# CSB5/lofreq

Hardware: AMD Instinct MI355X
Metric: pileup columns/sec at depth 10000 (higher is better)
Workload: dtype f64

## Files before the change

lofreq_amd/csrc/lfq_api.hip:

```cpp
#include "lfq_bound.h"
#include "lfq_ctx.h"

namespace {

struct LfqDeviceStreams {
    hipStream_t stream = nullptr, dps = nullptr, side[2] = {nullptr, nullptr};
    hipEvent_t ev_tail[3] = {nullptr, nullptr, nullptr};
    bool tail_recorded = false;
    hipEvent_t ev_end = nullptr;
    bool end_recorded = false;
    int refs = 0;
};
std::mutex g_streams_m;
LfqDeviceStreams g_streams[64];

bool acquire_streams(int device, lfq_ctx *c);
void release_streams(int device);

void *pin_acquire_impl(lfq_ctx *c, size_t bytes, int *slot)
{
    int best = -1, empty = -1, smallest = -1;
    for (int i = 0; i < LFQ_PIN_SLOTS; i++) {
        auto &b = c->pin_pool[i];
        if (b.used) {
// ... 230 lines not shown
    (void)hipSetDevice(c->device);
    for (;;) {
        {
            std::unique_lock<std::mutex> lk(*c->lm);
            c->lcv->wait(lk, [&] { return c->leader_go > 0 || c->leader_stop; });
            if (c->leader_stop) {
                return;
            }
            c->leader_go--;
        }
        int64_t n = 0;
        if (hipEventSynchronize(c->ev_heavy) == hipSuccess) {
            n = std::min<int64_t>(std::max<int64_t>(*(volatile int32_t *)c->h_nheavy, 0), c->heavy_cap);
        }
        lfq_sb_precompute(c->h_tuples, 3 * n);
        {
            std::lock_guard<std::mutex> lk(*c->lm);
            c->sb_pending--;
        }
        c->lcv->notify_all();
    }
}

int ensure_workspace(lfq_ctx *c, int64_t ncols)
{
    if (ncols > c->ws_cols) {
        int64_t cap = 0;
        int64_t want = ncols + ncols / 8 + 1024;
        if (c->d_flags) (void)hipFree(c->d_flags);
        if (c->d_prefix) (void)hipFree(c->d_prefix);
        if (c->d_entries) (void)hipFree(c->d_entries);
        if (c->d_tiles) (void)hipFree(c->d_tiles);
        if (c->d_unsplit) (void)hipFree(c->d_unsplit);
        if (c->d_retry) (void)hipFree(c->d_retry);
        c->d_unsplit = nullptr;
        c->d_retry = nullptr;
        c->d_flags = nullptr;
        c->d_prefix = nullptr;
        c->d_entries = nullptr;
        c->d_tiles = nullptr;
        c->ws_cols = 0;
        LFQ_TRY(grow(&c->d_flags, &cap, want));
        cap = 0;
        LFQ_TRY(grow(&c->d_prefix, &cap, want));
        cap = 0;
        LFQ_TRY(grow(&c->d_entries, &cap, want));
        cap = 0;
        LFQ_TRY(grow(&c->d_tiles, &cap, 2 * (want / 1024 + 8 * (LFQ_MAX_SEGMENTS + 1))));
        cap = 0;
        LFQ_TRY(grow(&c->d_unsplit, &cap, want));
        cap = 0;
        LFQ_TRY(grow(&c->d_retry, &cap, want));
        c->ws_cols = want;
    }
    return LFQ_OK;
}


}

void *lfq_pin_acquire(lfq_ctx *c, size_t bytes, int *slot) { return pin_acquire_impl(c, bytes, slot); }

extern "C" {

void *lfq_host_alloc(size_t bytes)
{
    void *p = nullptr;
    if (hipHostMalloc(&p, bytes ? bytes : 1, hipHostMallocDefault) != hipSuccess) {
        (void)hipGetLastError();
        return nullptr;
    }
    return p;
}

void lfq_host_free(void *p)
{
    if (p) {
        (void)hipHostFree(p);
    }
}
int lfq_create(lfq_ctx **out, int device_ordinal)
{
    if (!out) {
        return LFQ_ERR_INVALID;
    }
// ... 107 lines not shown
        }
        if (c->h_pin2) (void)hipHostFree(c->h_pin2);
        if (c->d_detlim) (void)hipFree(c->d_detlim);
        if (c->d_sites_in) (void)hipFree(c->d_sites_in);
        if (c->d_sites_out) (void)hipFree(c->d_sites_out);
        for (int i = 0; i < 4; i++) {
            if (c->ev_sites_t[i]) (void)hipEventDestroy(c->ev_sites_t[i]);
        }
        if (c->d_sum) (void)hipFree(c->d_sum);
        if (c->h_sum) (void)hipHostFree(c->h_sum);
        delete c->plp_sum;
        if (c->ev_sum_t[0]) (void)hipEventDestroy(c->ev_sum_t[0]);
        if (c->ev_sum_t[1]) (void)hipEventDestroy(c->ev_sum_t[1]);
        if (c->ev_baq_t[0]) (void)hipEventDestroy(c->ev_baq_t[0]);
        if (c->ev_baq_t[1]) (void)hipEventDestroy(c->ev_baq_t[1]);
        if (c->ev_idq_t[0]) (void)hipEventDestroy(c->ev_idq_t[0]);
        if (c->ev_idq_t[1]) (void)hipEventDestroy(c->ev_idq_t[1]);
        if (c->d_baq_scr) (void)hipFree(c->d_baq_scr);
        if (c->d_baq_expect) (void)hipFree(c->d_baq_expect);
        if (c->d_baq_tmp8) (void)hipFree(c->d_baq_tmp8);
        if (c->d_baq_nflag) (void)hipFree(c->d_baq_nflag);
        if (c->d_baq_itab) (void)hipFree(c->d_baq_itab);
        if (c->d_baq_terms) (void)hipFree(c->d_baq_terms);
        lfq_viterbi_release(c);
        if (c->h_tuples) (void)hipHostFree(c->h_tuples);
        if (c->h_nheavy) (void)hipHostFree(c->h_nheavy);
        if (c->ev_heavy) (void)hipEventDestroy(c->ev_heavy);
    }
    if (!c) {
        return;
    }
    (void)hipSetDevice(c->device);
    if (c->stream) (void)hipStreamSynchronize(c->stream);
    void *bufs[] = {c->d_luts, c->d_flags, c->d_prefix, c->d_entries, c->d_counters, c->d_tiles, c->d_longs, c->d_pool, c->d_unsplit, c->d_retry,
                    c->d_scratch, c->d_counts, c->d_pvals, c->d_stage, c->d_approx_mu};
    for (void *b : bufs) {
        if (b) (void)hipFree(b);
    }
    if (c->h_counters) (void)hipHostFree(c->h_counters);
    for (int i = 0; i < 4; i++) {
        if (c->ev[i]) (void)hipEventDestroy(c->ev[i]);
    }
    for (int i = 0; i < 3; i++) {
        if (c->ev_join[i]) (void)hipEventDestroy(c->ev_join[i]);
        if (i == 0 && c->ev_segw) (void)hipEventDestroy(c->ev_segw);
        if (i == 0 && c->ev_prep) (void)hipEventDestroy(c->ev_prep);
        if (i == 0 && c->ev_mid) (void)hipEventDestroy(c->ev_mid);
    }
    for (int s = 0; s < LFQ_MAX_SEGMENTS; s++) {
        hipEvent_t evs[] = {c->ev_cnt[s][0], c->ev_cnt[s][1], c->ev_scan[s], c->ev_light[s][0], c->ev_light[s][1],
                            c->ev_side[0][s][0], c->ev_side[0][s][1], c->ev_side[1][s][0], c->ev_side[1][s][1]};
        for (hipEvent_t e : evs) {
            if (e) (void)hipEventDestroy(e);
        }
    }
    if (c->own_streams) {
        release_streams(c->device);
    }
    free(c);
}

int lfq_synchronize(lfq_ctx *c)
{
    if (!c) {
        return LFQ_ERR_INVALID;
    }
    LFQ_TRY_HIP(hipStreamSynchronize(c->stream));
// ... 50 lines not shown
    LfqTracksDev T;
    T.nt = tr->nt;
    T.nt_packed = (tr->flags & LFQ_TRACKS_NT_PACKED) ? 1 : 0;
    T.pad_ = 0;
    T.bq = tr->bq;
    T.baq = tr->baq;
    T.mq = tr->mq;
    T.sq = tr->sq;
    T.col_off = tr->col_off;
    T.ref_base = tr->ref_base;
    T.coverage_plp = tr->coverage_plp;
    T.num_bases = tr->num_bases;
    T.ncols = tr->ncols;

    const int64_t ncols = tr->ncols;
    int32_t *gcounters = c->d_counters + LFQ_MAX_SEGMENTS * LFQ_NCOUNTERS;
    c->cur_stream = st;
    c->cur_pvals_cap = pvals_capacity;
    c->cur_ncols = ncols;
    c->cur_segments = 0;
    c->cur_col_off = tr->col_off;
    c->cur_indel_mode = indel_mode ? 1 : 0;
    c->cur_obs_bytes_x2 = (T.nt_packed ? 1 : 2) + 2;
    if (P.general) {
        c->cur_obs_bytes_x2 += 2 * ((T.baq ? 1 : 0) + 1 + (T.sq ? 1 : 0));
        if (P.def_alt_bq == -1) {
            c->cur_obs_bytes_x2 += (T.nt_packed ? 1 : 2) + 2;
        }
    }
    c->cur_col_bytes = 8 + 1 + (T.coverage_plp ? 4 : 0) + (T.num_bases ? 4 : 0) + (P.detlim_af ? 4 : 0);
    LFQ_TRY(lfq_order_after_batch(c, st));
    LFQ_TRY(tail_wait(c, st));
    LFQ_TRY_HIP(hipMemsetAsync(c->d_counters, 0, (LFQ_MAX_SEGMENTS + 1) * LFQ_NCOUNTERS * sizeof(int32_t), st));
    if (ncols > 0) {
        LFQ_TRY_HIP(hipMemsetAsync(c->d_retry, 0, (size_t)ncols, st));
    }
    LFQ_TRY_HIP(hipEventRecord(c->ev[0], st));
    if (ncols == 0) {
        LFQ_TRY_HIP(hipMemcpyAsync(c->h_counters, c->d_counters,
                                   (LFQ_MAX_SEGMENTS + 1) * LFQ_NCOUNTERS * sizeof(int32_t), hipMemcpyDeviceToHost, st));
        LFQ_TRY_HIP(hipEventRecord(c->ev[3], st));
        c->batch_recorded = 1;
        return LFQ_OK;
    }

    int64_t max_depth = tr->max_col_obs;
    if (max_depth <= 0) {
        LFQ_TRY(lfq_launch_maxdepth(T, gcounters, st));
        LFQ_TRY_HIP(hipMemcpyAsync(c->h_counters, gcounters, LFQ_NCOUNTERS * sizeof(int32_t), hipMemcpyDeviceToHost, st));
        LFQ_TRY_HIP(hipStreamSynchronize(st));
        max_depth = c->h_counters[LFQ_GC_MAXDEPTH];
    }
    {
        static const LfqLuts h_luts = [] {
            LfqLuts h;
            fill_luts(&h);
            return h;
        }();
        const bool lb = !P.general && P.def_alt_bq == 0 && P.def_alt_jp < 0.0;
        P.bound_p_lo = (lb && !indel_mode && kn.bound_gate && lfq_count_is_lean(T, P, max_depth))
                           ? lfq_bound_p_lo(h_luts.bq, P.min_alt_bq4, LFQ_BOUND_QLO) : 0.0;
    }
    const int64_t per_block = 3 * max_depth + 72;
    int n_big_blocks = c->n_cu;
    const int64_t budget = (int64_t)1 << 29;
    if (per_block * n_big_blocks > budget) {
        n_big_blocks = (int)std::max<int64_t>(8, budget / per_block);
    }
    LFQ_TRY(grow(&c->d_scratch, &c->scratch_doubles, per_block * n_big_blocks));
    if (!c->d_longs) {
        c->long_cap = 1 << 16;
        c->pool_cells = kn.split_pool_cells;
        LFQ_TRY_HIP(hipMalloc((void **)&c->d_longs, (size_t)c->long_cap * sizeof(LfqLong)));
        LFQ_TRY_HIP(hipMalloc((void **)&c->d_pool, (size_t)std::max(c->pool_cells, 1) * sizeof(LfqSegCell)));
        LFQ_TRY_HIP(hipEventCreateWithFlags(&c->ev_segw, hipEventDisableTiming));
        LFQ_TRY_HIP(hipEventCreateWithFlags(&c->ev_prep, hipEventDisableTiming));
        LFQ_TRY_HIP(hipEventCreateWithFlags(&c->ev_mid, hipEventDisableTiming));
    }

    const int n_seg = 1;
    c->cur_segments = n_seg;
    LFQ_TRY_HIP(hipEventRecord(c->ev_join[2], st));
    LFQ_TRY_HIP(hipStreamWaitEvent(dps, c->ev_join[2], 0));

    bool big_joined = false;
    for (int s = 0; s < n_seg; s++) {
        const int64_t c0 = ncols * s / n_seg, c1 = ncols * (s + 1) / n_seg;
        LfqWork W;
        W.tested_prefix = c->d_prefix;
        W.entries = c->d_entries + c0;
        W.counters = c->d_counters + s * LFQ_NCOUNTERS;
        W.gcounters = gcounters;
        W.block_sums = (int32_t *)(c->d_tiles + 2 * (c0 / 1024 + 8 * s));
        W.long_cap = c->long_cap / n_seg;
        W.pool_cells = c->pool_cells / n_seg;
        W.longs = c->d_longs + (int64_t)s * W.long_cap;
        W.pool = c->d_pool + (int64_t)s * W.pool_cells;
        W.unsplit = c->d_unsplit + c0;

        LFQ_TRY_HIP(hipEventRecord(c->ev_cnt[s][0], st));
        const bool ungated = c->batch_gate == LFQ_GATE_NONE && st == c->stream && !c->priv_stream_on && !single_stream;
        LFQ_TRY(lfq_launch_count(T, c0, c1, P, c->d_luts, d_counts, c->d_flags, max_depth, st, ungated));
        c->cur_sparse_counts = P.sparse_counts && lfq_count_is_shallow(T, P, max_depth);
        LFQ_TRY_HIP(hipEventRecord(c->ev_cnt[s][1], st));

        LFQ_TRY_HIP(hipStreamWaitEvent(dps, c->ev_cnt[s][1], 0));
        LFQ_TRY(lfq_launch_scan(T, c0, c1, c->d_flags, d_counts, W, dps));
        if (P.approx_n > 0) {
            LFQ_TRY(grow(&c->d_approx_mu, &c->approx_mu_bytes, (c1 - c0) * 8));
            LFQ_TRY(lfq_launch_approx_gate(T, P, c->d_luts, d_counts, W, c1 - c0, (double *)c->d_approx_mu, c->d_flags, dps));
            LFQ_TRY(lfq_launch_scan(T, c0, c1, c->d_flags, d_counts, W, dps, true));
        }
        LFQ_TRY_HIP(hipEventRecord(c->ev_scan[s], dps));
        const bool sb_heavy = n_seg == 1 && !indel_mode && c->leader && !kn.no_sb_precompute;
        auto launch_heavy = [&]() -> int {
            if (P.lazy_strand) {
                LFQ_TRY(lfq_launch_strand_heavy(T, W, d_counts, c->d_tuples_mapped, c->d_nheavy_mapped, c->heavy_cap, 16, dps));
            } else {
                LFQ_TRY(lfq_launch_gather_heavy(W, d_counts, c->d_tuples_mapped, c->d_nheavy_mapped, c->heavy_cap, 16, dps));
            }
            LFQ_TRY_HIP(hipEventRecord(c->ev_heavy, dps));
            {
                std::lock_guard<std::mutex> lk(*c->lm);
                c->leader_go++;
                c->sb_pending++;
            }
            c->lcv->notify_all();
            return LFQ_OK;
        };
        const bool screen = !kn.skip_light && kn.light_kernel != 2;
        if (sb_heavy && !screen) {
// ... 38 lines not shown
        }
        if (run_big) {
            LFQ_TRY(lfq_launch_dp_seg(1, T, P, c->d_luts, W, c->n_cu * 8, side0));
            LFQ_DBG_STAGE("seg big");
            LFQ_TRY(tail_record(c, 0, side0));
            LFQ_TRY(lfq_launch_dp_combine(1, P, d_counts, W, d_pvals, pvals_capacity, c->n_cu, side0));
            LFQ_DBG_STAGE("combine big");
            if (!big_on_st) {
                LFQ_TRY(lfq_launch_dp_big(T, P, c->d_luts, d_counts, W, d_pvals, pvals_capacity, c->d_scratch, per_block,
                                          n_big_blocks, side0));
                LFQ_DBG_STAGE("big");
            }
        }
        if (!run_big) {
            LFQ_TRY(tail_record(c, 0, side0));
        }
        LFQ_TRY_HIP(hipStreamWaitEvent(side1, c->ev_prep, 0));
        if (run_mid || run_big) {
            LFQ_TRY(lfq_launch_dp_seg(0, T, P, c->d_luts, W, c->n_cu * 8, side1));
            LFQ_DBG_STAGE("seg mid");
            LFQ_TRY(tail_record(c, 1, side1));
            LFQ_TRY(lfq_launch_dp_combine(0, P, d_counts, W, d_pvals, pvals_capacity, c->n_cu, side1));
            LFQ_DBG_STAGE("combine mid");
        }
        if (!(run_mid || run_big)) {
            LFQ_TRY(tail_record(c, 1, side1));
        }
        LFQ_TRY_HIP(hipEventRecord(c->ev_light[s][0], dps));
        if (!kn.skip_light) {
            if (kn.light_kernel == 2) {
                LFQ_TRY(lfq_launch_dp_light(T, P, c->d_luts, d_counts, W, d_pvals, pvals_capacity, n_light_waves, dps));
            } else {
                const int kh = indel_mode ? c->kreg_hint_indel : c->kreg_hint;
                LFQ_TRY(lfq_launch_dp_quad(T, P, c->d_luts, d_counts, W, c->d_retry + c0, d_pvals, pvals_capacity,
                                           n_light_waves, kh, dps, 1));
                LFQ_TRY(tail_record(c, 2, dps));
                if (sb_heavy) {
                    LFQ_TRY(launch_heavy());
                }
                LFQ_TRY(lfq_launch_dp_quad(T, P, c->d_luts, d_counts, W, c->d_retry + c0, d_pvals, pvals_capacity,
                                           n_light_waves, kh, dps, 2));
            }
        }
        LFQ_TRY_HIP(hipEventRecord(c->ev_light[s][1], dps));
        if (!screen) {
            LFQ_TRY(tail_record(c, 2, dps));
        }
        for (int i = 0; i < 2; i++) {
            LFQ_TRY_HIP(hipEventRecord(c->ev_side[i][s][1], side_i[i]));
        }
    }
    hipStream_t jn = (st != c->stream || single_stream) ? st : side0;
    LFQ_TRY_HIP(hipEventRecord(c->ev[1], st));
    LFQ_TRY_HIP(hipEventRecord(c->ev_join[0], side0));
    LFQ_TRY_HIP(hipEventRecord(c->ev_join[1], side1));
    LFQ_TRY_HIP(hipEventRecord(c->ev_join[2], dps));
    for (int i = 0; i < 3; i++) {
        LFQ_TRY_HIP(hipStreamWaitEvent(jn, c->ev_join[i], 0));
    }
    if (big_joined && jn != st) {
        LFQ_TRY_HIP(hipStreamWaitEvent(jn, c->ev_segw, 0));
    }
    if (P.lazy_strand && d_pvals && pvals_capacity > 0) {
        LFQ_TRY(lfq_launch_strand_pvals(T, d_pvals, gcounters + LFQ_GC_PVALS, pvals_capacity, c->n_cu, jn));
    }
    LFQ_TRY(end_record(c, jn));
    LFQ_TRY_HIP(hipMemcpyAsync(c->h_counters, c->d_counters, (LFQ_MAX_SEGMENTS + 1) * LFQ_NCOUNTERS * sizeof(int32_t),
                               hipMemcpyDeviceToHost, jn));
    {
        uint64_t *h_ends = reinterpret_cast<uint64_t *>(c->h_counters + (LFQ_MAX_SEGMENTS + 1) * LFQ_NCOUNTERS);
        if (c->cur_col_off) {
            LFQ_TRY_HIP(hipMemcpyAsync(h_ends, c->cur_col_off, 8, hipMemcpyDeviceToHost, jn));
            LFQ_TRY_HIP(hipMemcpyAsync(h_ends + 1, c->cur_col_off + c->cur_ncols, 8, hipMemcpyDeviceToHost, jn));
// ... 730 lines not shown
```

lofreq_amd/csrc/lfq_ctx.h:

```cpp
#ifndef LFQ_CTX_H
#define LFQ_CTX_H

#include <hip/hip_runtime.h>

#include <ctype.h>
#include <float.h>
#include <math.h>
#include <stdio.h>
#include <stdlib.h>
#include <string.h>

#include <algorithm>
#include <chrono>
#include <condition_variable>
#include <mutex>
#include <string>
#include <atomic>
#include <functional>
#include <unistd.h>
#include <fcntl.h>
#include <sys/file.h>
#include <thread>
#include <vector>

// ... 209 lines not shown
    std::vector<int32_t> n_ins, n_dels, hrun, cov;
    std::vector<char> key_chars;
};

#define LFQ_PIN_SLOTS 40

struct lfq_ctx {
    int device;
    hipStream_t stream;
    LfqLuts *d_luts;
    int64_t ws_cols;
    uint8_t *d_flags;
    uint8_t *d_approx_mu;
    int64_t approx_mu_bytes;
    int32_t *d_prefix, *d_counters;
    LfqEntry *d_entries;
    hipStream_t dps;
    hipStream_t side[2];
    hipEvent_t ev_mid;
    hipEvent_t ev_cnt[LFQ_MAX_SEGMENTS][2];
    hipEvent_t ev_scan[LFQ_MAX_SEGMENTS];
    hipEvent_t ev_light[LFQ_MAX_SEGMENTS][2];
    hipEvent_t ev_side[2][LFQ_MAX_SEGMENTS][2];
    hipEvent_t ev_join[3];
    int cur_segments;
    uint64_t *d_tiles;
    double *d_scratch;
    int64_t scratch_doubles;
    LfqLong *d_longs;
    LfqSegCell *d_pool;
    int32_t long_cap, pool_cells;
    hipEvent_t ev_segw, ev_prep;
    int32_t *d_unsplit;
    uint8_t *d_retry;
    int32_t *h_counters;
    lfq_col_counts *d_counts;
    int64_t counts_cap;
    lfq_col_pvals *d_pvals;
    int64_t pvals_cap;
    uint8_t *d_stage;
    int64_t stage_bytes;
    hipStream_t cur_stream;
    int64_t cur_pvals_cap;
    int64_t cur_ncols;
    hipEvent_t ev[4];
    lfq_kernel_times times;
    lfq_dp_work work;
    int64_t cur_count_read, cur_count_written;
    const uint64_t *cur_col_off;
    int cur_obs_bytes_x2, cur_col_bytes;
    int cur_sparse_counts;
    int n_cu;
    int32_t *h_tuples, *d_tuples_mapped;
    int32_t *h_nheavy, *d_nheavy_mapped;
    int heavy_cap;
    hipEvent_t ev_heavy;
    uint8_t *d_plp_in, *d_plp_out;
    int64_t plp_in_bytes, plp_out_bytes;
    uint8_t *d_tmp[5];
    struct { void *p; size_t cap; } rs_cache[7];
    int priv_stream_on;
    hipStream_t priv_stream;
    hipStream_t up_stream;
    hipEvent_t ev_up;
    hipEvent_t ev_apply;
    uint8_t *h_pin;
    int64_t pin_bytes;
// ... 145 lines not shown
```

lofreq_amd/csrc/lfq_dp.hip:

```cpp
#include <atomic>

#include "lfq_bound.h"
#include "lfq_device.h"

#define LFQ_LN2_HI 6.93147180369123816490e-01
#define LFQ_LN2_LO 1.90821492927058770002e-10
#define LFQ_EXP_UNDERFLOW_X (-708.3964185322641)
#define LFQ_DBL_EPS 2.220446049250313e-16

#ifndef LFQ_HEAVY_WAVES
#define LFQ_HEAVY_WAVES 8
#endif
#ifndef LFQ_DP512_WAVES
#define LFQ_DP512_WAVES 2
#endif

struct LfqColCtx {
    int col;
    uint64_t off0;
    int64_t n_obs;
    int ref_code;
    int median_ref_bq;
    int K;
    int64_t bonf;
// ... 850 lines not shown
        for (;;) {
            LfqColCtx cx;
            lfq_col_setup(cx, en, P);
            LfqRaw raw_next = raw;
            LfqEntry en_next2 = en_next;
            const bool have_next2 = have_next && (w + 2) < b1;
            LfqPrefetch pf;
            pf.want_raw = have_next;
            pf.off0 = en_next.off0;
            pf.n_obs = en_next.n_obs;
            pf.want_entry = have_next2;
            pf.entry_ptr = list + (have_next2 ? (w + 2) : w);
            pf.raw = &raw_next;
            pf.entry = &en_next2;
            if (MAXC == 1 || cx.K < 64) {
                lfq_wave_column<1, (MAXC > 1), (MAXC > 1)>(cx, raw, T, P, &s_luts, rows, counts, W, pvals, pvals_capacity, pf);
            } else {
                lfq_wave_column<4, true, true>(cx, raw, T, P, &s_luts, rows, counts, W, pvals, pvals_capacity, pf);
            }
            if (!have_next) {
                break;
            }
            w += 1;
            en = en_next;
            raw = raw_next;
            en_next = en_next2;
            have_next = have_next2;
        }
    }
}



__global__ __launch_bounds__(256) void lfq_dp_retry_kernel(LfqTracksDev T, LfqParams P,
                                                           const LfqLuts *__restrict__ g_luts,
                                                           const lfq_col_counts *__restrict__ counts, LfqWork W,
                                                           const uint8_t *__restrict__ retry,
                                                           lfq_col_pvals *__restrict__ pvals, int64_t pvals_capacity)
{
    __shared__ LfqLuts s_luts;
    __shared__ LfqRow s_rows[4][64];
    lfq_luts_to_lds(&s_luts, g_luts);
    __syncthreads();
    const int lane = lfq_lane();
    const int wave = __builtin_amdgcn_readfirstlane((int)(threadIdx.x >> 6));
    const int n_work = W.counters[LFQ_CNT_LIGHT];
    const int n_waves_total = (int)gridDim.x * 4;
    LfqRow *rows = s_rows[wave];
    for (int base = ((int)blockIdx.x * 4 + wave) * 16; base < n_work; base += n_waves_total * 16) {
        const int i = base + lane;
        uint64_t m = __ballot(lane < 16 && i < n_work && retry[i] != 0);
        while (m != 0ull) {
            const int j = __builtin_ctzll(m);
            m &= m - 1ull;
            const LfqEntry en = lfq_load_entry(W.entries, base + j);
            LfqColCtx cx;
            lfq_col_setup(cx, en, P);
            const LfqRaw raw = lfq_load_chunk_at(en.off0, en.n_obs, 0, T);
            LfqPrefetch pf;
            pf.want_raw = false;
            pf.want_entry = false;
            pf.off0 = 0;
            pf.n_obs = 0;
            pf.entry_ptr = nullptr;
            pf.raw = nullptr;
            pf.entry = nullptr;
            lfq_wave_column<1, true, false>(cx, raw, T, P, &s_luts, rows, counts, W, pvals, pvals_capacity, pf);
        }
    }
}


template <int KREG>
__device__ __forceinline__ void lfq_screen_row(double (&v)[KREG], double p, double q)
{
    v[KREG - 1] = fma(v[KREG - 2], p, v[KREG - 1]);
#pragma unroll
    for (int j = KREG - 2; j >= 1; j--) {
        v[j] = fma(v[j - 1], p, v[j] * q);
    }
    v[0] = v[0] * q;
}

#define LFQ_SCREEN_BYTE(w4, j) \
    (((((j) >> 2) == 0 ? (w4).x : ((j) >> 2) == 1 ? (w4).y : ((j) >> 2) == 2 ? (w4).z : (w4).w) >> (8 * ((j) & 3))) & 0xffu)

#define LFQ_SCREEN_CLAIM 128

template <int KREG, bool LB, bool GATE>
__global__ __launch_bounds__(256) void lfq_dp_screen_kernel(LfqTracksDev T, LfqParams P,
                                                            const LfqLuts *__restrict__ g_luts, LfqWork W,
                                                            uint8_t *__restrict__ retry, int max_rounds)
{
    constexpr int MAXK = KREG - 1;
    static_assert(MAXK <= LFQ_BOUND_MAXK, "the bound gate's table");
    static_assert(LB || !GATE, "the bound needs the LB conditions");
    __shared__ LfqLuts s_luts;
    __shared__ LfqBoundTab s_bound;
    lfq_luts_to_lds(&s_luts, g_luts);
    if constexpr (GATE) {
        if (threadIdx.x < LFQ_BOUND_CODES) {
            s_bound.qm[threadIdx.x] = lfq_bound_qm(P.bound_p_lo, threadIdx.x);
        } else if (threadIdx.x >= 64 && threadIdx.x < 64 + LFQ_BOUND_NRK) {
            s_bound.rk[threadIdx.x - 64] = lfq_bound_rk(P.bound_p_lo, (int)threadIdx.x - 64);
        }
    }
    __syncthreads();
    const int lane = lfq_lane();
    const int n_work = W.counters[LFQ_CNT_LIGHT];
    const LfqEntry *list = W.entries;
    const double sig_s = P.sig * (1.0 + P.prune_slack);
    const LfqEvalMasks EM = lfq_eval_masks(P);
    const int xcd0 = (int)(blockIdx.x & 7u);
    int xcd_try = 0;
    int q_next = 0, q_end = 0;

    bool active = false;
    uint64_t off0 = 0;
    int n_obs = 0, rel = 0, K = 0, ref_code = 0, med = 0, rounds = 0, list_idx = 0, n_kept = 0;
    double bonf_d = 1.0;
    double v[KREG];
#pragma unroll
    for (int j = 0; j < KREG; j++) {
        v[j] = 0.0;
    }
    unsigned long long acc_cells = 0, acc_rows = 0;
    int n_retry = 0;

    for (;;) {
        uint64_t need = __ballot(!active);
        while (need != 0ull && (q_next < q_end || xcd_try < 8)) {
            if (q_next >= q_end) {
                const int x = (xcd0 + xcd_try) & 7;
                const int lo = (int)((int64_t)n_work * x / 8), hi = (int)((int64_t)n_work * (x + 1) / 8);
                int32_t *head = &W.counters[LFQ_CNT_XHEAD + 32 * x];
                int b = __hip_atomic_load(head, __ATOMIC_RELAXED, __HIP_MEMORY_SCOPE_AGENT);
                if (b < hi - lo) {
                    b = lfq_claim(head, LFQ_SCREEN_CLAIM);
                }
                if (b >= hi - lo) {
                    xcd_try++;
                    continue;
                }
                q_next = lo + b;
                q_end = min(lo + b + LFQ_SCREEN_CLAIM, hi);
            }
            const int idx = q_next + __popcll(need & ((1ull << lane) - 1ull));
            q_next = min(q_next + __popcll(need), q_end);
            if (!active && idx < q_end) {
                const uint4 *ep = reinterpret_cast<const uint4 *>(list + idx);
                const uint4 a = ep[0], b = ep[1];
                K = (int)b.y;
                if (K > MAXK) {
                    retry[idx] = 1;
                    n_retry++;
                } else {
                    int64_t bonf = P.bonf_base;
                    if (P.bonf_dynamic) {
                        bonf = ((P.bonf_reset_first && P.bonf_base == 1) ? 0 : P.bonf_base)
                               + (int64_t)P.bonf_step * (int)b.x;
                    }
                    bonf_d = (double)bonf;
                    active = true;
                    if constexpr (GATE) {
                        active = !(b.w != 0u && lfq_bound_tail(&s_bound, b.w & (LFQ_BOUND_CODES - 1u), K) * bonf_d > sig_s);
                    }
                    off0 = ((uint64_t)a.y << 32) | a.x;
                    n_obs = (int)a.z;
                    med = (int)(int16_t)(b.z & 0xffffu);
                    ref_code = (int)((b.z >> 16) & 0xffu);
                    rel = -(int)(off0 & 15u);
                    rounds = 0;
                    n_kept = 0;
                    list_idx = idx;
#pragma unroll
                    for (int j = 0; j < KREG; j++) {
                        v[j] = (j == MAXK - K) ? 1.0 : 0.0;
                    }
                }
            }
            need = __ballot(!active);
        }
        if (__ballot(active) == 0ull) {
            break;
        }

        uint4 bqw = make_uint4(0, 0, 0, 0), baqw = make_uint4(~0u, ~0u, ~0u, ~0u), mqw = make_uint4(0, 0, 0, 0);
        uint4 sqw = make_uint4(~0u, ~0u, ~0u, ~0u), ntw = make_uint4(0, 0, 0, 0);
        if (active) {
            const uint64_t wbase = (uint64_t)((int64_t)off0 + rel);
            bqw = *reinterpret_cast<const uint4 *>(T.bq + wbase);
            mqw = *reinterpret_cast<const uint4 *>(T.mq + wbase);
            if (!LB && T.baq) {
                baqw = *reinterpret_cast<const uint4 *>(T.baq + wbase);
            }
            if (!LB && T.sq) {
                sqw = *reinterpret_cast<const uint4 *>(T.sq + wbase);
            }
            if (T.nt_packed) {
                const uint2 n2 = *reinterpret_cast<const uint2 *>(T.nt + (wbase >> 1));
                ntw.x = n2.x;
                ntw.y = n2.y;
            } else {
                ntw = *reinterpret_cast<const uint4 *>(T.nt + wbase);
            }
        }
        const bool packed = T.nt_packed != 0;
#pragma unroll
        for (int j = 0; j < 16; j++) {
            const uint32_t nib = (((j >> 3) ? ntw.y : ntw.x) >> (8 * (j & 3) + 4 * ((j & 7) >> 2))) & 15u;
            const uint32_t ntb = packed ? nib : LFQ_SCREEN_BYTE(ntw, j);
            if (LB) {
                const uint32_t code = ntb & 7u, bqb = LFQ_SCREEN_BYTE(bqw, j);
                const bool valid = code <= 3u;
                const bool is_alt = valid & (code != (uint32_t)ref_code);
                const bool bq_ok = (int)bqb >= (is_alt ? P.min_alt_bq4 : P.min_bq4);
                const double pm = s_luts.mq[LFQ_SCREEN_BYTE(mqw, j) | EM.off_mq];
                const double pl = fma(1.0 - pm, s_luts.bq[bqb], pm);
                const bool keep = active & valid & bq_ok & ((unsigned)(rel + j) < (unsigned)n_obs);
                lfq_screen_row<KREG>(v, keep ? pl : 0.0, keep ? 1.0 - pl : 1.0);
                n_kept += keep ? 1 : 0;
                continue;
            }
            const LfqObs o = lfq_eval_obs_flat(ntb, LFQ_SCREEN_BYTE(bqw, j), LFQ_SCREEN_BYTE(baqw, j), LFQ_SCREEN_BYTE(mqw, j),
                                               LFQ_SCREEN_BYTE(sqw, j), ref_code, med, P, EM, &s_luts);
            const bool keep = active & o.keep & ((unsigned)(rel + j) < (unsigned)n_obs);
            const double ps = fmax(o.p, LFQ_DBL_EPS);
            const double qf = fmax(1.0 - o.p, LFQ_DBL_EPS);
            lfq_screen_row<KREG>(v, keep ? ps : 0.0, keep ? qf : 1.0);
            n_kept += keep ? 1 : 0;
        }
        rel += 16;
        rounds += 1;
        if (active) {
            const bool pruned = v[KREG - 1] * bonf_d > sig_s;
            const bool give_up = !pruned && (rel >= n_obs || rounds >= max_rounds);
            if (pruned || give_up) {
                active = false;
                acc_cells += lfq_cells_of(n_kept, K);
                acc_rows += (unsigned long long)n_kept;
                if (give_up) {
                    retry[list_idx] = 1;
                    n_retry++;
                }
            }
        }
    }
#pragma unroll
    for (int d = 32; d >= 1; d >>= 1) {
        acc_cells += __shfl_xor(acc_cells, d, 64);
        acc_rows += __shfl_xor(acc_rows, d, 64);
        n_retry += __shfl_xor(n_retry, d, 64);
    }
    if (lane == 0 && acc_rows) {
        atomicAdd(reinterpret_cast<unsigned long long *>(W.gcounters + LFQ_GC_CELLS), acc_cells);
        atomicAdd(reinterpret_cast<unsigned long long *>(W.gcounters + LFQ_GC_ROWS), acc_rows);
    }
    if (lane == 0 && n_retry) {
        atomicAdd(&W.gcounters[LFQ_GC_SCREEN_RETRY], n_retry);
    }
}


struct LfqBigShared {
    LfqLuts luts;
    LfqRow rows[LFQ_HEAVY_WAVES][64];
    double bv[2][LFQ_HEAVY_WAVES][128];
    int be[2][LFQ_HEAVY_WAVES][128];
    double zero_v[64];
    int zero_e[64];
    double gv[LFQ_HEAVY_WAVES][64];
    int ge[LFQ_HEAVY_WAVES][64];
    double mu[LFQ_HEAVY_WAVES];
    int col, pruned, split;
};

__device__ __forceinline__ void lfq_big_bounds_impl(const LfqColCtx &cx, const lfq_col_counts &cnt,
                                                    const LfqTracksDev &T, const LfqParams &P, const LfqLuts *luts,
                                                    double *mu_sh, int NW, unsigned *uf_mask_out, double *uf_bound,
                                                    int *kp_out)
{
    const int lane = lfq_lane();
    const int w = __builtin_amdgcn_readfirstlane((int)(threadIdx.x >> 6));
    const int64_t n_chunks = (cx.n_obs + 63) / 64;
    double part = 0.0;
// ... 1433 lines not shown
    {
        static std::atomic<unsigned long long> allowed{0ull};
        int dev = 0;
        if (hipGetDevice(&dev) != hipSuccess) {
            return LFQ_ERR_HIP;
        }
        const unsigned long long bit = 1ull << (dev & 63);
        if (!(allowed.load(std::memory_order_acquire) & bit)) {
            const int bytes = (int)sizeof(LfqCombShared);
            if (hipFuncSetAttribute(reinterpret_cast<const void *>(&lfq_dp_combine_kernel<0>),
                                    hipFuncAttributeMaxDynamicSharedMemorySize, bytes) != hipSuccess ||
                hipFuncSetAttribute(reinterpret_cast<const void *>(&lfq_dp_combine_kernel<1>),
                                    hipFuncAttributeMaxDynamicSharedMemorySize, bytes) != hipSuccess) {
                return LFQ_ERR_HIP;
            }
            allowed.fetch_or(bit, std::memory_order_release);
        }
    }
    if (mode == 0) {
        hipLaunchKernelGGL(lfq_dp_fold_kernel<0>, dim3((unsigned)n_blocks * 4), dim3(64 * LFQ_FOLD_WAVES), 0,
                           (hipStream_t)stream, p, d_counts, w, d_pvals, pvals_capacity);
        hipLaunchKernelGGL(lfq_dp_combine_kernel<0>, dim3((unsigned)n_blocks), dim3(LFQ_COMB_THREADS), sizeof(LfqCombShared),
                           (hipStream_t)stream, p, d_counts, w, d_pvals, pvals_capacity, 1);
    } else {
        hipLaunchKernelGGL(lfq_dp_fold_kernel<1>, dim3((unsigned)n_blocks), dim3(64 * LFQ_FOLD_WAVES), 0,
                           (hipStream_t)stream, p, d_counts, w, d_pvals, pvals_capacity);
        hipLaunchKernelGGL(lfq_dp_combine_kernel<1>, dim3((unsigned)n_blocks), dim3(LFQ_COMB_THREADS), sizeof(LfqCombShared),
                           (hipStream_t)stream, p, d_counts, w, d_pvals, pvals_capacity, 1);
    }
    return hipGetLastError() == hipSuccess ? LFQ_OK : LFQ_ERR_HIP;
}

int lfq_launch_dp_quad(const LfqTracksDev &t, const LfqParams &p, const LfqLuts *d_luts,
                       const lfq_col_counts *d_counts, const LfqWork &w, uint8_t *d_retry, lfq_col_pvals *d_pvals,
                       int64_t pvals_capacity, int n_waves, int kreg_hint, void *stream, int phase)
{
    if (t.ncols <= 0 || n_waves <= 0) {
        return LFQ_OK;
    }
    const dim3 grid((unsigned)((n_waves + 3) / 4)), block(256);
    hipStream_t st = (hipStream_t)stream;
    const LfqKnobs &kn = lfq_knobs();
    int force = 0;
    if (phase != 2) {
        if (!force) {
            force = kreg_hint > 0 ? kreg_hint : 8;
        }
        const bool lb = !p.general && p.def_alt_bq == 0 && p.def_alt_jp < 0.0;
#define LFQ_LAUNCH_SCREEN(KR)                                                                                        \
    do {                                                                                                             \
        if (lb && p.bound_p_lo > 0.0) {                                                                              \
            hipLaunchKernelGGL((lfq_dp_screen_kernel<KR, true, true>), grid, block, 0, st, t, p, d_luts, w, d_retry, \
                               kn.screen_rounds);                                                                    \
        } else if (lb) {                                                                                             \
            hipLaunchKernelGGL((lfq_dp_screen_kernel<KR, true, false>), grid, block, 0, st, t, p, d_luts, w, d_retry, \
                               kn.screen_rounds);                                                                    \
        } else {                                                                                                     \
            hipLaunchKernelGGL((lfq_dp_screen_kernel<KR, false, false>), grid, block, 0, st, t, p, d_luts, w, d_retry, \
                               kn.screen_rounds);                                                                    \
        }                                                                                                            \
    } while (0)
        if (force <= 6) LFQ_LAUNCH_SCREEN(6);
        else if (force <= 8) LFQ_LAUNCH_SCREEN(8);
        else if (force <= 10) LFQ_LAUNCH_SCREEN(10);
        else if (force <= 12) LFQ_LAUNCH_SCREEN(12);
        else if (force <= 16) LFQ_LAUNCH_SCREEN(16);
        else if (force <= 24) LFQ_LAUNCH_SCREEN(24);
        else if (force <= 32) LFQ_LAUNCH_SCREEN(32);
        else {
            hipLaunchKernelGGL(lfq_dp_wave_kernel<1>, grid, block, 0, st, t, p, d_luts, d_counts, w, -1, LFQ_CNT_LIGHT,
                               d_pvals, pvals_capacity, 32, 0);
        }
#undef LFQ_LAUNCH_SCREEN
    }
    if (phase != 1) {
        hipLaunchKernelGGL(lfq_dp_retry_kernel, grid, block, 0, st, t, p, d_luts, d_counts, w, d_retry, d_pvals,
                           pvals_capacity);
    }
    return hipGetLastError() == hipSuccess ? LFQ_OK : LFQ_ERR_HIP;
}
```

lofreq_amd/csrc/lfq_internal.h:

```cpp
#ifndef LFQ_INTERNAL_H
#define LFQ_INTERNAL_H

#include <stdint.h>

#include "lofreq_amd.h"

struct LfqLuts {
    double bq[256];
    double baq[256];
    double mq[256];
    double sq[256];
};

struct LfqParams {
    int32_t min_bq4;
    int32_t min_alt_bq4;
    int32_t def_alt_bq;
    int32_t general;
    double jq_reject_above;
    double alt_jq_reject_above;
    double def_alt_jp;
    int32_t min_cov;
    int32_t use_baq, use_mq, use_sq;
    int32_t bonf_dynamic;
// ... 63 lines not shown
    int32_t pad1_;
    double uf_bound[3];
    int64_t pad_[4];
};

#define LFQ_SEG_MAX 8
#define LFQ_SEG_CLASSES 5
#define LFQ_SEG_MIN_CHUNKS 16
#ifndef LFQ_SEG_MIN_CHUNKS_SHORT
#define LFQ_SEG_MIN_CHUNKS_SHORT 4
#endif
#define LFQ_SEG_SHORT_BELOW 48
#define LFQ_PHASE1_CHUNKS 8
#define LFQ_SEG_BUDGET 4096
#define LFQ_SPLIT_MAX_K 2016

#if defined(__HIPCC__)
__host__ __device__
#endif
static inline int lfq_khist_thr(int f)
{
    return f == 0 ? 5 : f == 1 ? 7 : f == 2 ? 9 : f == 3 ? 11 : f == 4 ? 15 : f == 5 ? 23 : 31;
}

struct LfqWork {
    int32_t *tested_prefix;
    LfqEntry *entries;
    int32_t *gcounters;
    int32_t *counters;
    int32_t *block_sums;
    LfqLong *longs;
    int32_t *unsplit;
    LfqSegCell *pool;
    int32_t long_cap;
    int32_t pool_cells;
};

#define LFQ_MID_K 64
#define LFQ_BIG_K 250
#define LFQ_NCOUNTERS 320
#define LFQ_MAX_SEGMENTS 1
#define LFQ_GC_PVALS 0
#define LFQ_GC_OVERFLOW 1
#define LFQ_GC_TESTED 2
#define LFQ_GC_MAXDEPTH 3
#define LFQ_GC_CELLS 8
#define LFQ_GC_ROWS 10
#define LFQ_GC_APPROX_PRUNED 13
#define LFQ_GC_SCREEN_RETRY 12
#define LFQ_CNT_TESTED 0
#define LFQ_CNT_BIG 1
#define LFQ_CNT_MID 2
#define LFQ_CNT_LIGHT 3
#define LFQ_CNT_HEAD 4
#define LFQ_CNT_CARRY_IN 15
#define LFQ_CNT_HEAD_LIGHT 12
#define LFQ_CNT_HEAD_MID 13
#define LFQ_CNT_UNSPLIT 5
#define LFQ_CNT_HEAD_PREP 6
#define LFQ_CNT_POOL 7
#define LFQ_CNT_HEAD_COMB 24
#define LFQ_CNT_HEAD_FOLD 48
#define LFQ_CNT_KLE7 26
#define LFQ_CNT_KLE15 27
#define LFQ_CNT_KLE31 28
#define LFQ_CNT_XHEAD 64
#define LFQ_CNT_KHIST 40
#define LFQ_NKHIST 7
#define LFQ_CNT_LONG0 16

#define LFQ_SEQ_LETTERS "ACGTN=MRSVWYHKDB"
#if defined(__HIPCC__)
__host__ __device__
#endif
static inline char lfq_seq_letter(unsigned code)
{
    return code > 15u ? 'N' : LFQ_SEQ_LETTERS[code];
}

struct LfqKnobs {
    int timing;
    int single_stream;
    int no_sb_precompute;
    int debug_sync;
    int skip_light, skip_mid, skip_big;
    int light_kernel;
    int screen_rounds;
    int seg_max;
    int seg_max_mid;
    int split_pool_cells;
    long count_multi_below;
    int big_on_side;
    int baq_one_variant;
    int pileup_tiles;
    long host_loop_threads;
    long count_lpg4_below, count_lpg8_below;
    long host_spin_us;
    int sync_upload;
    int host_threads;
// ... 196 lines not shown
    const uint8_t *seq, *qual;
    const char *ref;
    int64_t ref_len;
    const uint8_t *ign;
    int32_t nonmatch_qual, min_bq;
    double *scratch;
    int64_t scratch_cells;
    double *prob;
    uint8_t *status;
};
int lfq_launch_srcq(const LfqSrcqArgs &a, const LfqLuts *d_luts, int n_blocks, void *stream);
int lfq_launch_pileup_scatter(const LfqPileupArgs &a, void *stream);

int lfq_launch_strand_heavy(const LfqTracksDev &t, const LfqWork &w, lfq_col_counts *d_counts, int32_t *tuples_mapped,
                            int32_t *n_mapped, int cap_entries, int min_alt, void *stream);
int lfq_launch_strand_pvals(const LfqTracksDev &t, lfq_col_pvals *d_pvals, const int32_t *d_n_pvals, int64_t cap, int n_blocks,
                            void *stream);
int lfq_launch_gather_heavy(const LfqWork &w, const lfq_col_counts *d_counts, int32_t *tuples_mapped,
                            int32_t *n_mapped, int cap_entries, int min_alt, void *stream);
int lfq_launch_maxdepth(const LfqTracksDev &t, int32_t *d_gcounters, void *stream);
int lfq_launch_ntcount(const LfqTracksDev &t, int32_t *d_out, void *stream);
bool lfq_count_is_shallow(const LfqTracksDev &t, const LfqParams &p, int64_t max_col_obs);
int lfq_launch_count(const LfqTracksDev &t, int64_t c0, int64_t c1, const LfqParams &p, const LfqLuts *d_luts,
                     lfq_col_counts *d_counts, uint8_t *d_flags, int64_t max_col_obs, void *stream, bool shallow_half_cu = false);
bool lfq_count_is_lean(const LfqTracksDev &t, const LfqParams &p, int64_t max_col_obs);
int lfq_launch_scan(const LfqTracksDev &t, int64_t c0, int64_t c1, const uint8_t *d_flags,
                    const lfq_col_counts *d_counts, const LfqWork &w, void *stream, bool relist = false);
int lfq_launch_approx_gate(const LfqTracksDev &t, const LfqParams &p, const LfqLuts *d_luts, const lfq_col_counts *d_counts,
                           const LfqWork &w, int64_t ncols_seg, double *d_mu, uint8_t *d_flags, void *stream);
int lfq_launch_dp_light(const LfqTracksDev &t, const LfqParams &p, const LfqLuts *d_luts,
                        const lfq_col_counts *d_counts, const LfqWork &w, lfq_col_pvals *d_pvals,
                        int64_t pvals_capacity, int n_waves, void *stream);
int lfq_launch_dp_quad(const LfqTracksDev &t, const LfqParams &p, const LfqLuts *d_luts,
                       const lfq_col_counts *d_counts, const LfqWork &w, uint8_t *d_retry, lfq_col_pvals *d_pvals,
                       int64_t pvals_capacity, int n_waves, int kreg_hint, void *stream, int phase = 0);
int lfq_launch_dp_mid(const LfqTracksDev &t, const LfqParams &p, const LfqLuts *d_luts,
                      const lfq_col_counts *d_counts, const LfqWork &w, lfq_col_pvals *d_pvals,
                      int64_t pvals_capacity, int n_waves, void *stream);
int lfq_launch_dp_big(const LfqTracksDev &t, const LfqParams &p, const LfqLuts *d_luts,
                      const lfq_col_counts *d_counts, const LfqWork &w, lfq_col_pvals *d_pvals,
                      int64_t pvals_capacity, double *d_scratch, int64_t scratch_doubles_per_block,
                      int n_blocks, void *stream);
int lfq_launch_dp_big_prep(const LfqTracksDev &t, const LfqParams &p, const LfqLuts *d_luts,
                           const lfq_col_counts *d_counts, const LfqWork &w, lfq_col_pvals *d_pvals,
                           int64_t pvals_capacity, int n_blocks, void *stream);
int lfq_launch_dp_seg(int mode, const LfqTracksDev &t, const LfqParams &p, const LfqLuts *d_luts,
                      const LfqWork &w, int n_waves, void *stream);
int lfq_launch_dp_combine(int mode, const LfqParams &p, const lfq_col_counts *d_counts, const LfqWork &w,
                          lfq_col_pvals *d_pvals, int64_t pvals_capacity, int n_blocks, void *stream);
int lfq_launch_synth(const struct lfq_synth_spec *d_spec_host, int64_t col_begin, int64_t ncols,
                     uint8_t *d_nt, uint8_t *d_bq, uint8_t *d_baq, uint8_t *d_mq, uint64_t *d_col_off,
                     uint8_t *d_ref_base, int nt_packed, void *stream);

#endif
```

Measured before the change: 363.8 million.

## Replace dense retry flag array with compacted retry list via wave-aggregated atomics

The screen kernel now appends retry column indices to a compact list with one wave-aggregated atomic per wave, replacing per-column byte flags. The retry kernel walks only that list, one column per wave, instead of scanning every light entry's flag, and exits early when the list is empty. This also removes the per-batch memset of the flag array. In exchange, retry order is no longer sorted by index, atomics are added in the screen loop, and the counter block grows.

Result: no change. 364.4 million, median of 3 (+0.2%).

```diff
diff --git a/lofreq_amd/csrc/lfq_api.hip b/lofreq_amd/csrc/lfq_api.hip
--- a/lofreq_amd/csrc/lfq_api.hip
+++ b/lofreq_amd/csrc/lfq_api.hip
@@ -286,9 +286,9 @@
         if (c->d_entries) (void)hipFree(c->d_entries);
         if (c->d_tiles) (void)hipFree(c->d_tiles);
         if (c->d_unsplit) (void)hipFree(c->d_unsplit);
-        if (c->d_retry) (void)hipFree(c->d_retry);
+        if (c->d_retry_list) (void)hipFree(c->d_retry_list);
         c->d_unsplit = nullptr;
-        c->d_retry = nullptr;
+        c->d_retry_list = nullptr;
         c->d_flags = nullptr;
         c->d_prefix = nullptr;
         c->d_entries = nullptr;
@@ -304,7 +304,7 @@
         cap = 0;
         LFQ_TRY(grow(&c->d_unsplit, &cap, want));
         cap = 0;
-        LFQ_TRY(grow(&c->d_retry, &cap, want));
+        LFQ_TRY(grow(&c->d_retry_list, &cap, want));
         c->ws_cols = want;
     }
     return LFQ_OK;
@@ -478,7 +478,7 @@
     }
     (void)hipSetDevice(c->device);
     if (c->stream) (void)hipStreamSynchronize(c->stream);
-    void *bufs[] = {c->d_luts, c->d_flags, c->d_prefix, c->d_entries, c->d_counters, c->d_tiles, c->d_longs, c->d_pool, c->d_unsplit, c->d_retry,
+    void *bufs[] = {c->d_luts, c->d_flags, c->d_prefix, c->d_entries, c->d_counters, c->d_tiles, c->d_longs, c->d_pool, c->d_unsplit, c->d_retry_list,
                     c->d_scratch, c->d_counts, c->d_pvals, c->d_stage, c->d_approx_mu};
     for (void *b : bufs) {
         if (b) (void)hipFree(b);
@@ -595,9 +595,6 @@
     LFQ_TRY(lfq_order_after_batch(c, st));
     LFQ_TRY(tail_wait(c, st));
     LFQ_TRY_HIP(hipMemsetAsync(c->d_counters, 0, (LFQ_MAX_SEGMENTS + 1) * LFQ_NCOUNTERS * sizeof(int32_t), st));
-    if (ncols > 0) {
-        LFQ_TRY_HIP(hipMemsetAsync(c->d_retry, 0, (size_t)ncols, st));
-    }
     LFQ_TRY_HIP(hipEventRecord(c->ev[0], st));
     if (ncols == 0) {
         LFQ_TRY_HIP(hipMemcpyAsync(c->h_counters, c->d_counters,
@@ -660,6 +657,7 @@
         W.longs = c->d_longs + (int64_t)s * W.long_cap;
         W.pool = c->d_pool + (int64_t)s * W.pool_cells;
         W.unsplit = c->d_unsplit + c0;
+        W.retry_list = c->d_retry_list + c0;
 
         LFQ_TRY_HIP(hipEventRecord(c->ev_cnt[s][0], st));
         const bool ungated = c->batch_gate == LFQ_GATE_NONE && st == c->stream && !c->priv_stream_on && !single_stream;
@@ -764,13 +762,13 @@
                 LFQ_TRY(lfq_launch_dp_light(T, P, c->d_luts, d_counts, W, d_pvals, pvals_capacity, n_light_waves, dps));
             } else {
                 const int kh = indel_mode ? c->kreg_hint_indel : c->kreg_hint;
-                LFQ_TRY(lfq_launch_dp_quad(T, P, c->d_luts, d_counts, W, c->d_retry + c0, d_pvals, pvals_capacity,
+                LFQ_TRY(lfq_launch_dp_quad(T, P, c->d_luts, d_counts, W, d_pvals, pvals_capacity,
                                            n_light_waves, kh, dps, 1));
                 LFQ_TRY(tail_record(c, 2, dps));
                 if (sb_heavy) {
                     LFQ_TRY(launch_heavy());
                 }
-                LFQ_TRY(lfq_launch_dp_quad(T, P, c->d_luts, d_counts, W, c->d_retry + c0, d_pvals, pvals_capacity,
+                LFQ_TRY(lfq_launch_dp_quad(T, P, c->d_luts, d_counts, W, d_pvals, pvals_capacity,
                                            n_light_waves, kh, dps, 2));
             }
         }
diff --git a/lofreq_amd/csrc/lfq_ctx.h b/lofreq_amd/csrc/lfq_ctx.h
--- a/lofreq_amd/csrc/lfq_ctx.h
+++ b/lofreq_amd/csrc/lfq_ctx.h
@@ -265,7 +265,7 @@
     int32_t long_cap, pool_cells;
     hipEvent_t ev_segw, ev_prep;
     int32_t *d_unsplit;
-    uint8_t *d_retry;
+    int32_t *d_retry_list;
     int32_t *h_counters;
     lfq_col_counts *d_counts;
     int64_t counts_cap;
diff --git a/lofreq_amd/csrc/lfq_dp.hip b/lofreq_amd/csrc/lfq_dp.hip
--- a/lofreq_amd/csrc/lfq_dp.hip
+++ b/lofreq_amd/csrc/lfq_dp.hip
@@ -906,41 +906,54 @@
 
 
 
+__device__ __forceinline__ int lfq_retry_append(const LfqWork &W, bool flag, int idx)
+{
+    const uint64_t m = __ballot(flag);
+    if (m == 0ull) {
+        return 0;
+    }
+    const int lane = lfq_lane(), n = __popcll(m), leader = __builtin_ctzll(m);
+    int base = 0;
+    if (lane == leader) {
+        base = atomicAdd(&W.counters[LFQ_CNT_RETRY_N], n);
+    }
+    base = __shfl(base, leader, 64);
+    if (flag) {
+        W.retry_list[base + __popcll(m & ((1ull << lane) - 1ull))] = idx;
+    }
+    return n;
+}
+
 __global__ __launch_bounds__(256) void lfq_dp_retry_kernel(LfqTracksDev T, LfqParams P,
                                                            const LfqLuts *__restrict__ g_luts,
                                                            const lfq_col_counts *__restrict__ counts, LfqWork W,
-                                                           const uint8_t *__restrict__ retry,
                                                            lfq_col_pvals *__restrict__ pvals, int64_t pvals_capacity)
 {
     __shared__ LfqLuts s_luts;
     __shared__ LfqRow s_rows[4][64];
+    const int n_retry = W.counters[LFQ_CNT_RETRY_N];
+    if (n_retry <= 0) {
+        return;
+    }
     lfq_luts_to_lds(&s_luts, g_luts);
     __syncthreads();
-    const int lane = lfq_lane();
     const int wave = __builtin_amdgcn_readfirstlane((int)(threadIdx.x >> 6));
-    const int n_work = W.counters[LFQ_CNT_LIGHT];
     const int n_waves_total = (int)gridDim.x * 4;
     LfqRow *rows = s_rows[wave];
-    for (int base = ((int)blockIdx.x * 4 + wave) * 16; base < n_work; base += n_waves_total * 16) {
-        const int i = base + lane;
-        uint64_t m = __ballot(lane < 16 && i < n_work && retry[i] != 0);
-        while (m != 0ull) {
-            const int j = __builtin_ctzll(m);
-            m &= m - 1ull;
-            const LfqEntry en = lfq_load_entry(W.entries, base + j);
-            LfqColCtx cx;
-            lfq_col_setup(cx, en, P);
-            const LfqRaw raw = lfq_load_chunk_at(en.off0, en.n_obs, 0, T);
-            LfqPrefetch pf;
-            pf.want_raw = false;
-            pf.want_entry = false;
-            pf.off0 = 0;
-            pf.n_obs = 0;
-            pf.entry_ptr = nullptr;
-            pf.raw = nullptr;
-            pf.entry = nullptr;
-            lfq_wave_column<1, true, false>(cx, raw, T, P, &s_luts, rows, counts, W, pvals, pvals_capacity, pf);
-        }
+    for (int i = (int)blockIdx.x * 4 + wave; i < n_retry; i += n_waves_total) {
+        const LfqEntry en = lfq_load_entry(W.entries, W.retry_list[i]);
+        LfqColCtx cx;
+        lfq_col_setup(cx, en, P);
+        const LfqRaw raw = lfq_load_chunk_at(en.off0, en.n_obs, 0, T);
+        LfqPrefetch pf;
+        pf.want_raw = false;
+        pf.want_entry = false;
+        pf.off0 = 0;
+        pf.n_obs = 0;
+        pf.entry_ptr = nullptr;
+        pf.raw = nullptr;
+        pf.entry = nullptr;
+        lfq_wave_column<1, true, false>(cx, raw, T, P, &s_luts, rows, counts, W, pvals, pvals_capacity, pf);
     }
 }
 
@@ -963,8 +976,7 @@
 
 template <int KREG, bool LB, bool GATE>
 __global__ __launch_bounds__(256) void lfq_dp_screen_kernel(LfqTracksDev T, LfqParams P,
-                                                            const LfqLuts *__restrict__ g_luts, LfqWork W,
-                                                            uint8_t *__restrict__ retry, int max_rounds)
+                                                            const LfqLuts *__restrict__ g_luts, LfqWork W, int max_rounds)
 {
     constexpr int MAXK = KREG - 1;
     static_assert(MAXK <= LFQ_BOUND_MAXK, "the bound gate's table");
@@ -1021,13 +1033,13 @@
             }
             const int idx = q_next + __popcll(need & ((1ull << lane) - 1ull));
             q_next = min(q_next + __popcll(need), q_end);
+            bool wide = false;
             if (!active && idx < q_end) {
                 const uint4 *ep = reinterpret_cast<const uint4 *>(list + idx);
                 const uint4 a = ep[0], b = ep[1];
                 K = (int)b.y;
                 if (K > MAXK) {
-                    retry[idx] = 1;
-                    n_retry++;
+                    wide = true;
                 } else {
                     int64_t bonf = P.bonf_base;
                     if (P.bonf_dynamic) {
@@ -1053,6 +1065,7 @@
                     }
                 }
             }
+            n_retry += lfq_retry_append(W, wide, idx);
             need = __ballot(!active);
         }
         if (__ballot(active) == 0ull) {
@@ -1106,25 +1119,22 @@
         }
         rel += 16;
         rounds += 1;
+        bool give_up = false;
         if (active) {
             const bool pruned = v[KREG - 1] * bonf_d > sig_s;
-            const bool give_up = !pruned && (rel >= n_obs || rounds >= max_rounds);
+            give_up = !pruned && (rel >= n_obs || rounds >= max_rounds);
             if (pruned || give_up) {
                 active = false;
                 acc_cells += lfq_cells_of(n_kept, K);
                 acc_rows += (unsigned long long)n_kept;
-                if (give_up) {
-                    retry[list_idx] = 1;
-                    n_retry++;
-                }
-            }
-        }
+            }
+        }
+        n_retry += lfq_retry_append(W, give_up, list_idx);
     }
 #pragma unroll
     for (int d = 32; d >= 1; d >>= 1) {
         acc_cells += __shfl_xor(acc_cells, d, 64);
         acc_rows += __shfl_xor(acc_rows, d, 64);
-        n_retry += __shfl_xor(n_retry, d, 64);
     }
     if (lane == 0 && acc_rows) {
         atomicAdd(reinterpret_cast<unsigned long long *>(W.gcounters + LFQ_GC_CELLS), acc_cells);
@@ -2624,7 +2634,7 @@
 }
 
 int lfq_launch_dp_quad(const LfqTracksDev &t, const LfqParams &p, const LfqLuts *d_luts,
-                       const lfq_col_counts *d_counts, const LfqWork &w, uint8_t *d_retry, lfq_col_pvals *d_pvals,
+                       const lfq_col_counts *d_counts, const LfqWork &w, lfq_col_pvals *d_pvals,
                        int64_t pvals_capacity, int n_waves, int kreg_hint, void *stream, int phase)
 {
     if (t.ncols <= 0 || n_waves <= 0) {
@@ -2642,13 +2652,13 @@
 #define LFQ_LAUNCH_SCREEN(KR)                                                                                        \
     do {                                                                                                             \
         if (lb && p.bound_p_lo > 0.0) {                                                                              \
-            hipLaunchKernelGGL((lfq_dp_screen_kernel<KR, true, true>), grid, block, 0, st, t, p, d_luts, w, d_retry, \
+            hipLaunchKernelGGL((lfq_dp_screen_kernel<KR, true, true>), grid, block, 0, st, t, p, d_luts, w,          \
                                kn.screen_rounds);                                                                    \
         } else if (lb) {                                                                                             \
-            hipLaunchKernelGGL((lfq_dp_screen_kernel<KR, true, false>), grid, block, 0, st, t, p, d_luts, w, d_retry, \
+            hipLaunchKernelGGL((lfq_dp_screen_kernel<KR, true, false>), grid, block, 0, st, t, p, d_luts, w,          \
                                kn.screen_rounds);                                                                    \
         } else {                                                                                                     \
-            hipLaunchKernelGGL((lfq_dp_screen_kernel<KR, false, false>), grid, block, 0, st, t, p, d_luts, w, d_retry, \
+            hipLaunchKernelGGL((lfq_dp_screen_kernel<KR, false, false>), grid, block, 0, st, t, p, d_luts, w,          \
                                kn.screen_rounds);                                                                    \
         }                                                                                                            \
     } while (0)
@@ -2666,8 +2676,7 @@
 #undef LFQ_LAUNCH_SCREEN
     }
     if (phase != 1) {
-        hipLaunchKernelGGL(lfq_dp_retry_kernel, grid, block, 0, st, t, p, d_luts, d_counts, w, d_retry, d_pvals,
-                           pvals_capacity);
+        hipLaunchKernelGGL(lfq_dp_retry_kernel, grid, block, 0, st, t, p, d_luts, d_counts, w, d_pvals, pvals_capacity);
     }
     return hipGetLastError() == hipSuccess ? LFQ_OK : LFQ_ERR_HIP;
 }
diff --git a/lofreq_amd/csrc/lfq_internal.h b/lofreq_amd/csrc/lfq_internal.h
--- a/lofreq_amd/csrc/lfq_internal.h
+++ b/lofreq_amd/csrc/lfq_internal.h
@@ -119,13 +119,14 @@
     LfqLong *longs;
     int32_t *unsplit;
     LfqSegCell *pool;
+    int32_t *retry_list;
     int32_t long_cap;
     int32_t pool_cells;
 };
 
 #define LFQ_MID_K 64
 #define LFQ_BIG_K 250
-#define LFQ_NCOUNTERS 320
+#define LFQ_NCOUNTERS 352
 #define LFQ_MAX_SEGMENTS 1
 #define LFQ_GC_PVALS 0
 #define LFQ_GC_OVERFLOW 1
@@ -152,6 +153,7 @@
 #define LFQ_CNT_KLE15 27
 #define LFQ_CNT_KLE31 28
 #define LFQ_CNT_XHEAD 64
+#define LFQ_CNT_RETRY_N 320
 #define LFQ_CNT_KHIST 40
 #define LFQ_NKHIST 7
 #define LFQ_CNT_LONG0 16
@@ -414,7 +416,7 @@
                         const lfq_col_counts *d_counts, const LfqWork &w, lfq_col_pvals *d_pvals,
                         int64_t pvals_capacity, int n_waves, void *stream);
 int lfq_launch_dp_quad(const LfqTracksDev &t, const LfqParams &p, const LfqLuts *d_luts,
-                       const lfq_col_counts *d_counts, const LfqWork &w, uint8_t *d_retry, lfq_col_pvals *d_pvals,
+                       const lfq_col_counts *d_counts, const LfqWork &w, lfq_col_pvals *d_pvals,
                        int64_t pvals_capacity, int n_waves, int kreg_hint, void *stream, int phase = 0);
 int lfq_launch_dp_mid(const LfqTracksDev &t, const LfqParams &p, const LfqLuts *d_luts,
                       const lfq_col_counts *d_counts, const LfqWork &w, lfq_col_pvals *d_pvals,
```
